# dgrzech/sobfu

Hardware: AMD Instinct MI355X
Metric: solver iterations/sec on 256^3 voxel grid (higher is better)
Workload: dtype f32

## Files before the change

### sobfu_amd/csrc/sobfu_launch.hpp

```cpp
#pragma once
#include <hip/hip_runtime.h>

#include <cstddef>
#include <cstdint>

namespace sobfu_hip {
struct LaunchBox {
    int x0, x1, y0, y1, z0, z1;
    bool direct;
};
struct TileLaunchBox {
    LaunchBox box;
    float* dst;
    int ox, oy, oz, px, py;
    int push_y0, push_y1, local_z0, local_z1;
};
int launch_pass_a_boxes(const float* pnp, const float* pg, const float* psi, float* nU, float w_reg, int X, int Y, int Z, const LaunchBox* boxes,
                        int n, const uint32_t* prev_slots, float max_update_norm, int zc, hipStream_t stream, bool compact);
constexpr int kMaxSync = 64;
struct TileSync {
    uint32_t ticket_push, reserved;
    uint64_t wait_ticks;
    uint32_t wait_count, pad0;
    uint32_t err;
    uint32_t n_sync;
    uint32_t my_rank, world;
    uint64_t timeout_ticks;
    uint32_t* my_flags;
    uint32_t* my_grows;
    int sync_rank[kMaxSync];
    uint32_t* peer_flags[kMaxSync];
    uint32_t* peer_grows[kMaxSync];
};
struct TilePassAPlan;
int tile_pass_a_plan_create(TilePassAPlan** out, const TileLaunchBox* boxes, int n, int X, int Y, int Z);
void tile_pass_a_plan_destroy(TilePassAPlan* p);
int launch_tile_pass_a_plan(const TilePassAPlan* p, const float* pnp, const float* pg, const float* psi, float* nU, float w_reg, TileSync* sync,
                            uint32_t seq, int wait, const uint32_t* row, uint32_t row_index, hipStream_t stream);
int launch_tile_flush(TileSync* sync, uint32_t seq, int wait, const uint32_t* row, uint32_t row_index, hipStream_t stream);
int launch_tile_pingpong(TileSync* sync, int q, int first, uint32_t seq0, int reps, hipStream_t stream);
int launch_pass_b_boxes(const float* nU, float* psi, const float* phi_n, float* pnp, float* updates, uint32_t* slots, const float taps[7],
                        float alpha, int X, int Y, int Z, int pX, int pY, int pZ, const int own[6], const LaunchBox* boxes, int n,
                        const uint32_t* prev_slots, float max_update_norm, int zc, hipStream_t stream, bool compact,
                        float* psi_out = nullptr , int prev_rows = 1,
                        bool sys_acquire = false );
int launch_pass_a(const float* pnp, const float* pg, const float* psi, float* nU, float w_reg, int X, int Y, int Z,
                  const uint32_t* prev_slots, float max_update_norm, int zc, hipStream_t stream, bool compact, int z_lo = 0, int z_hi = 0,
                  int z_lo2 = 0, int z_hi2 = 0);
int launch_pass_b(const float* nU, float* psi, const float* phi_n, float* pnp, float* updates, uint32_t* slots,
                  const float taps[7], float alpha, int X, int Y, int Z, const uint32_t* prev_slots,
                  float max_update_norm, int zc, hipStream_t stream, int phi_Z, int own_lo, int own_hi, bool compact, int z_lo = 0,
                  int z_hi = 0, int z_lo2 = 0, int z_hi2 = 0, float* psi_out = nullptr ,
                  int prev_rows = 1 );
int launch_pack_vec(const float* src4, float* dst3, size_t N, hipStream_t stream);
int launch_unpack_vec(const float* src3, float* dst4, size_t N, hipStream_t stream);
int launch_extract_tsdf(const float* src2, float* dst1, size_t N, hipStream_t stream);
int launch_apply_tsdf_only(const float* phi1, float* out1, const float* psi3, int X, int Y, int Z, hipStream_t stream, int phi_Z = 0, int phi_X = 0,
                           int phi_Y = 0);
int launch_msg_copy(bool pack, float* field3, float* buf, int Lx, int Ly, int Lz, const int* boxes, int n, hipStream_t stream);
int launch_msg_scatter_table(float* field3, const float* buf, const uint32_t* d_table, unsigned n_cells, hipStream_t stream);
int launch_compact_enter(const float* psi4, const float* pg2, const float* pn2, float* c_psi, float* c_g, float* c_n, float* c_f, int X, int Y,
                         int Z, hipStream_t stream);
int launch_compact_leave(const float* c_psi, const float* pn2, float* psi4, float* pnp2, int X, int Y, int Z, hipStream_t stream);
int data_energy_tsdf(const float* g1, const float* f1, int n, void* d_scratch, float* out, hipStream_t stream);
int reg_energy_from_psi3(const float* psi3, int X, int Y, int Z, void* d_scratch, float* out, hipStream_t stream);
}
```

### sobfu_amd/csrc/solver_capi.hip

```cpp
#include <algorithm>
#include <cmath>
#include <cstdio>
#include <cstdlib>
#include <cstring>
#include <string>
#include <vector>

#include "sobfu_device.hpp"
#include "sobfu_hip.h"
#include "sobfu_host.hpp"
#include "sobfu_launch.hpp"


namespace {

constexpr int kSlots      = 256;
constexpr int kCheckEvery = 32;
constexpr int kMaxRunAhead = 96;

float host_sqrt_rd(float s) {
    float r = std::sqrt(s);
    if (r > 0.f && (double) r * (double) r > (double) s) r = std::nextafterf(r, -INFINITY);
    return r;
}

float slots_to_norm(const uint32_t* s) {
    uint32_t m = 0;
    for (int i = 0; i < kSlots; ++i) m = s[i] > m ? s[i] : m;
    float f;
    std::memcpy(&f, &m, 4);
    return host_sqrt_rd(f);
}

}

struct sobfu_hip_solver {
    int X = 0, Y = 0, Z = 0;
    size_t N = 0;
    sobfu_hip_solver_params p{};
    float taps[7]{};
    float* nabla_U     = nullptr;
    float* updates     = nullptr;
    float* c_psi = nullptr;
    float* c_f   = nullptr;
    float* c_g   = nullptr;
    float* c_n   = nullptr;
    bool compact = true;
    uint32_t* slots    = nullptr;
    uint32_t* h_rows   = nullptr;
    int h_rows_iters   = 0;
    hipEvent_t ev_chk  = nullptr;
    void* red_scratch  = nullptr;
    int slots_iters    = 0;
    bool keep_updates  = false;
    sobfu_hip_log_fn log_fn = nullptr;
    void* log_user          = nullptr;
    bool log_set            = false;
    size_t bytes            = 0;
    int prof_stride = 0;
    std::vector<hipEvent_t> events;
    double ms_a = 0, ms_b = 0;
    int prof_launches = 0, prof_pending = 0;
    struct Session {
        bool active = false, compact = false;
        const float *pg = nullptr, *pn = nullptr;
        float *pnp = nullptr, *psi = nullptr;
        const float *it_pnp = nullptr, *it_pg = nullptr, *it_pn = nullptr;
        float *it_psi = nullptr, *it_out = nullptr, *upd = nullptr;
        int cap = 0;
        int launched = 0;
        int checked = 0, fl_to = 0;
        bool in_flight = false;
        int done = 0;
        bool converged = false;
        float last_norm = 0.f;
        bool inline_log = false;
    } q;

    void log(const std::string& line) const {
        if (log_set) {
            if (log_fn) log_fn(line.c_str(), log_user);
        } else {
            std::printf("%s\n", line.c_str());
        }
    }
};

namespace {

std::string fmt_g(float v) {
    char b[64];
    std::snprintf(b, sizeof b, "%g", (double) v);
    return b;
}

int ensure_slots(sobfu_hip_solver* s, int iters) {
    if (iters <= s->slots_iters) return 0;
    if (s->slots) {
        SOBFU_HIP_TRY(hipFree(s->slots));
        s->bytes -= (size_t) (s->slots_iters + 1) * kSlots * 4;
    }
    s->slots = nullptr;
    SOBFU_HIP_TRY(hipMalloc((void**) &s->slots, (size_t) (iters + 1) * kSlots * 4));
    s->slots_iters = iters;
    s->bytes += (size_t) (iters + 1) * kSlots * 4;
    return 0;
}

int ensure_poll(sobfu_hip_solver* s, int iters) {
    if (!s->ev_chk) SOBFU_HIP_TRY(hipEventCreateWithFlags(&s->ev_chk, hipEventDisableTiming));
    if (iters <= s->h_rows_iters) return 0;
    if (s->h_rows) SOBFU_HIP_TRY(hipHostFree(s->h_rows));
    s->h_rows = nullptr;
    SOBFU_HIP_TRY(hipHostMalloc((void**) &s->h_rows, (size_t) iters * kSlots * 4, hipHostMallocDefault));
    s->h_rows_iters = iters;
    return 0;
}

int ensure_compact(sobfu_hip_solver* s) {
    if (s->c_psi) return 0;
    SOBFU_HIP_TRY(hipMalloc((void**) &s->c_psi, s->N * 12));
    SOBFU_HIP_TRY(hipMalloc((void**) &s->c_f, s->N * 4));
    SOBFU_HIP_TRY(hipMalloc((void**) &s->c_g, s->N * 4));
    SOBFU_HIP_TRY(hipMalloc((void**) &s->c_n, s->N * 4));
    s->bytes += s->N * 24;
    return 0;
}

int ensure_updates(sobfu_hip_solver* s) {
    if (s->updates) return 0;
    SOBFU_HIP_TRY(hipMalloc((void**) &s->updates, s->N * 16));
    s->bytes += s->N * 16;
    return 0;
}

int set_params(sobfu_hip_solver* s, const sobfu_hip_solver_params* p) {
    SOBFU_CHECK_ARGS(p && p->max_iter >= 0);
    if (p->s < 7 || p->s > 16) return p->s < 7 ? SOBFU_E_UNSUPPORTED : SOBFU_E_FILTER;
    float h[16];
    SOBFU_TRY(sobfu_hip_sobolev_filter(p->s, p->lambda, h));
    for (int i = 0; i < 7; ++i) s->taps[i] = h[i];
    s->p = *p;
    return 0;
}

int ensure_events(sobfu_hip_solver* s, size_t n) {
    while (s->events.size() < n) {
        hipEvent_t e;
        SOBFU_HIP_TRY(hipEventCreate(&e));
        s->events.push_back(e);
    }
    return 0;
}

int session_begin_impl(sobfu_hip_solver* s, const float* pg, const float* pn, float* pnp, float* psi, int cap, hipStream_t st) {
    sobfu_hip_solver::Session& q = s->q;
    const int X = s->X, Y = s->Y, Z = s->Z;
    q = sobfu_hip_solver::Session{};
    q.pg = pg; q.pn = pn; q.pnp = pnp; q.psi = psi;
    q.cap = cap;
    q.compact = s->compact && cap > 0;
    q.last_norm = NAN;
    if (!q.compact) SOBFU_TRY(sobfu_hip_apply(pn, pnp, psi, X, Y, Z, st));
    if (cap <= 0) return 0;
    SOBFU_TRY(ensure_slots(s, cap));
    SOBFU_HIP_TRY(hipMemsetAsync(s->slots, 0, (size_t) (cap + 1) * kSlots * 4, st));
    if (s->keep_updates) {
        SOBFU_TRY(ensure_updates(s));
        q.upd = s->updates;
    }
    q.it_pnp = pnp; q.it_pg = pg; q.it_pn = pn; q.it_psi = psi; q.it_out = pnp;
    if (q.compact) {
        SOBFU_TRY(ensure_compact(s));
        SOBFU_TRY(sobfu_hip::launch_compact_enter(psi, pg, pn, s->c_psi, s->c_g, s->c_n, s->c_f, X, Y, Z, st));
        q.it_pnp = s->c_f; q.it_pg = s->c_g; q.it_pn = s->c_n; q.it_psi = s->c_psi; q.it_out = s->c_f;
    }
    if (s->p.max_update_norm >= 0.f) SOBFU_TRY(ensure_poll(s, cap));
    if (s->prof_stride > 0) SOBFU_TRY(ensure_events(s, (size_t) 3 * (cap / s->prof_stride + 1)));
    return 0;
}
int session_begin(sobfu_hip_solver* s, const float* pg, const float* pn, float* pnp, float* psi, int cap, hipStream_t st) {
    if (s->q.active) return SOBFU_E_BADARG;
    const int rc = session_begin_impl(s, pg, pn, pnp, psi, cap, st);
    s->q.active = rc == 0;
    return rc;
}

void session_examine(sobfu_hip_solver* s, int upto, float* per_iter) {
    sobfu_hip_solver::Session& q = s->q;
    for (int k = q.checked; k < upto && !q.converged; ++k) {
        const float v = slots_to_norm(s->h_rows + (size_t) k * kSlots);
        if (per_iter) per_iter[k] = v;
        q.last_norm = v;
        q.done = k + 1;
        if (v <= s->p.max_update_norm) q.converged = true;
    }
    q.checked = upto;
}

int session_enqueue(sobfu_hip_solver* s, int n, bool poll, float* per_iter, hipStream_t st) {
    sobfu_hip_solver::Session& q = s->q;
    if (!q.active || n < 0 || q.launched + n > q.cap) return SOBFU_E_BADARG;
    const int X = s->X, Y = s->Y, Z = s->Z;
    const sobfu_hip_solver_params& p = s->p;
    const bool can_converge = p.max_update_norm >= 0.f;
    const int last = q.launched + n;
    for (int it = q.launched + 1; it <= last && !q.converged; ++it) {
        const uint32_t* prev = (it > 1) ? s->slots + (size_t) (it - 1) * kSlots : nullptr;
        uint32_t* cur        = s->slots + (size_t) it * kSlots;
        const bool ev = s->prof_stride > 0 && (it % s->prof_stride == 0) && (size_t) 3 * (s->prof_pending + 1) <= s->events.size();
        const int e0  = 3 * s->prof_pending;
        if (ev) SOBFU_HIP_TRY(hipEventRecord(s->events[e0], st));
        SOBFU_TRY(sobfu_hip::launch_pass_a(q.it_pnp, q.it_pg, q.it_psi, s->nabla_U, p.w_reg, X, Y, Z, prev, p.max_update_norm, 0, st, q.compact));
        if (ev) SOBFU_HIP_TRY(hipEventRecord(s->events[e0 + 1], st));
        SOBFU_TRY(sobfu_hip::launch_pass_b(s->nabla_U, q.it_psi, q.it_pn, q.it_out, q.upd, cur, s->taps, p.alpha, X, Y, Z, prev,
                                           p.max_update_norm, 0, st, 0, 0, 0, q.compact));
        if (ev) {
            SOBFU_HIP_TRY(hipEventRecord(s->events[e0 + 2], st));
            s->prof_pending += 1;
        }
        q.launched = it;
        if (can_converge && poll) {
            if (!q.in_flight && (it % kCheckEvery == 0 || it == last)) {
                SOBFU_HIP_TRY(hipMemcpyAsync(s->h_rows + (size_t) q.checked * kSlots, s->slots + (size_t) (q.checked + 1) * kSlots,
                                             (size_t) (it - q.checked) * kSlots * 4, hipMemcpyDeviceToHost, st));
                SOBFU_HIP_TRY(hipEventRecord(s->ev_chk, st));
                q.in_flight = true;
                q.fl_to     = it;
            }
            if (q.in_flight) {
                const bool must_wait = it - q.checked >= kMaxRunAhead;
                hipError_t e = must_wait ? hipEventSynchronize(s->ev_chk) : hipEventQuery(s->ev_chk);
                if (e == hipSuccess) {
                    session_examine(s, q.fl_to, per_iter);
                    q.in_flight = false;
                } else if (e != hipErrorNotReady) {
                    return (int) e;
                }
            }
        }
    }
    return 0;
}

int session_drain(sobfu_hip_solver* s, float* per_iter, hipStream_t st) {
    sobfu_hip_solver::Session& q = s->q;
    if (q.launched == 0) return 0;
    if (s->p.max_update_norm >= 0.f) {
        if (q.in_flight) {
            SOBFU_HIP_TRY(hipEventSynchronize(s->ev_chk));
            session_examine(s, q.fl_to, per_iter);
            q.in_flight = false;
        }
        if (!q.converged && q.checked < q.launched) {
            SOBFU_HIP_TRY(hipMemcpyAsync(s->h_rows + (size_t) q.checked * kSlots, s->slots + (size_t) (q.checked + 1) * kSlots,
                                         (size_t) (q.launched - q.checked) * kSlots * 4, hipMemcpyDeviceToHost, st));
            SOBFU_HIP_TRY(hipStreamSynchronize(st));
            session_examine(s, q.launched, per_iter);
        }
    } else {
        std::vector<uint32_t> hs((size_t) q.launched * kSlots);
        SOBFU_HIP_TRY(hipMemcpyAsync(hs.data(), s->slots + kSlots, hs.size() * 4, hipMemcpyDeviceToHost, st));
        SOBFU_HIP_TRY(hipStreamSynchronize(st));
        for (int k = 0; k < q.launched; ++k) {
            const float v = slots_to_norm(hs.data() + (size_t) k * kSlots);
            if (per_iter) per_iter[k] = v;
            q.last_norm = v;
        }
        q.done = q.launched;
    }
    return 0;
}

int session_end(sobfu_hip_solver* s, sobfu_hip_solver_report* rep, float* per_iter, hipStream_t st) {
    sobfu_hip_solver::Session& q = s->q;
    if (!q.active) return SOBFU_E_BADARG;
    sobfu_hip_solver_report r{};
    r.last_max_update_norm = NAN;
    r.last_max_update_index = NAN;
    r.last_e_data = r.last_e_reg = NAN;
    SOBFU_TRY(session_drain(s, per_iter, st));
    if (q.compact) SOBFU_TRY(sobfu_hip::launch_compact_leave(s->c_psi, q.pn, q.psi, q.pnp, s->X, s->Y, s->Z, st));
    for (int it = 1; it <= q.done && !q.inline_log; ++it)
        if (it == 1 || it % 50 == 0) s->log("iter. no. " + std::to_string(it));
    if (q.converged) s->log("SOLVER CONVERGED AFTER " + std::to_string(q.done) + " ITERATIONS");
    else if (q.cap > 0 && q.done == q.cap) s->log("SOLVER REACHED MAX. NO. OF ITERATIONS WITHOUT CONVERGING");
    r.iterations = q.done;
    r.converged  = q.converged ? 1 : 0;
    r.last_max_update_norm = q.last_norm;
    q.active = false;
    SOBFU_HIP_TRY(hipStreamSynchronize(st));
    if (rep) *rep = r;
    return 0;
}

int run_verbose(sobfu_hip_solver* s, const float* pg, const float* pn, float* pnp, float* psi, int max_iter,
                sobfu_hip_solver_report* rep, float* per_iter, hipStream_t st) {
    const int X = s->X, Y = s->Y, Z = s->Z;
    const sobfu_hip_solver_params& p = s->p;
    auto reports = [&](int it) { return p.verbosity == 2 || (p.verbosity == 1 && (it == 1 || it % 50 == 0 || it == max_iter)); };
    SOBFU_TRY(ensure_updates(s));
    SOBFU_TRY(session_begin(s, pg, pn, pnp, psi, max_iter, st));
    sobfu_hip_solver::Session& q = s->q;
    q.upd = s->updates;
    q.inline_log = p.verbosity <= 2;
    float e_data = NAN, e_reg = NAN, arg = NAN;
    auto fail = [&](int rc) {
        q.active = false;
        return rc;
    };
#define SOBFU_VTRY(expr)                    \
    do {                                    \
        const int rc_ = (int) (expr);       \
        if (rc_ != 0) return fail(rc_);     \
    } while (0)
    for (int it = 1; it <= max_iter && !q.converged;) {
        if (!reports(it)) {
            int to = it;
            while (to + 1 <= max_iter && !reports(to + 1)) ++to;
            SOBFU_VTRY(session_enqueue(s, to - it + 1, true, per_iter, st));
            if (p.max_update_norm >= 0.f) SOBFU_VTRY(session_drain(s, per_iter, st));
            it = to + 1;
            continue;
        }
        if (it == 1 || it % 50 == 0) s->log("iter. no. " + std::to_string(it));
        if (q.compact) {
            SOBFU_VTRY(sobfu_hip::data_energy_tsdf(q.it_pg, q.it_pnp, (int) s->N, s->red_scratch, &e_data, st));
            SOBFU_VTRY(sobfu_hip::reg_energy_from_psi3(q.it_psi, X, Y, Z, s->red_scratch, &e_reg, st));
        } else {
            SOBFU_VTRY(sobfu_hip_data_energy(pg, pnp, (int) s->N, s->red_scratch, &e_data, st));
            SOBFU_VTRY(sobfu_hip_reg_energy_sobolev_from_psi(psi, X, Y, Z, s->red_scratch, &e_reg, st));
        }
        const float e = e_data + p.w_reg * e_reg;
        s->log("data energy + w_reg * reg energy = " + fmt_g(e_data) + " + " + fmt_g(p.w_reg) + " * " + fmt_g(e_reg) + " = " + fmt_g(e));
        uint32_t* cur = s->slots + (size_t) it * kSlots;
        SOBFU_VTRY(sobfu_hip::launch_pass_a(q.it_pnp, q.it_pg, q.it_psi, s->nabla_U, p.w_reg, X, Y, Z, nullptr, 0.f, 0, st, q.compact));
        SOBFU_VTRY(sobfu_hip::launch_pass_b(s->nabla_U, q.it_psi, q.it_pn, q.it_out, s->updates, cur, s->taps, p.alpha, X, Y, Z, nullptr, 0.f, 0, st, 0,
                                            0, 0, q.compact));
        float mx[2];
        SOBFU_VTRY(sobfu_hip_max_update_norm(s->updates, (int) s->N, s->red_scratch, mx, st));
        if (per_iter) per_iter[it - 1] = mx[0];
        arg = mx[1];
        q.launched = q.checked = q.done = it;
        q.last_norm = mx[0];
        {
            int ix = (int) (mx[1] / (float) (X * Y));
            int iy = (int) ((mx[1] - (float) (ix * X * Y)) / (float) X);
            int iz = (int) (mx[1] - (float) (X * (iy + Y * ix)));
            s->log("max. update norm " + fmt_g(mx[0]) + " at voxel (" + std::to_string(iz) + ", " + std::to_string(iy) + ", " + std::to_string(ix) + ")");
        }
        if (mx[0] <= p.max_update_norm) q.converged = true;
        ++it;
    }
#undef SOBFU_VTRY
    const bool last_reported = q.done > 0 && reports(q.done);
    sobfu_hip_solver_report r{};
    SOBFU_TRY(session_end(s, &r, per_iter, st));
    r.last_e_data = e_data;
    r.last_e_reg  = e_reg;
    r.last_max_update_index = last_reported ? arg : NAN;
    if (rep) *rep = r;
    return 0;
}

int run_loop(sobfu_hip_solver* s, const float* pg, const float* pn, float* pnp, float* psi, int max_iter,
             sobfu_hip_solver_report* rep, float* per_iter, hipStream_t st) {
    if (s->q.active) return SOBFU_E_BADARG;
    if (s->p.verbosity > 0 && max_iter > 0) return run_verbose(s, pg, pn, pnp, psi, max_iter, rep, per_iter, st);
    SOBFU_TRY(session_begin(s, pg, pn, pnp, psi, max_iter, st));
// ... 192 lines not shown
```

### sobfu_amd/csrc/solver_kernels.hip

```cpp
#include <algorithm>
#include <cstdlib>
#include <vector>

#include "sobfu_device.hpp"
#include "sobfu_hip.h"
#include "sobfu_host.hpp"
#include "sobfu_launch.hpp"

using namespace sobfu_hip;

#ifndef SOBFU_SWIZZLE_B
#define SOBFU_SWIZZLE_B true
#endif

namespace {

struct Taps {
    float s[7];
};
constexpr int kMaxMsgs = 18;

#include "solver_iter_common.inl"
#include "solver_pass_a.inl"
#include "solver_pass_b.inl"
#include "solver_aux_kernels.inl"

}

constexpr int kRPT = 1, kWY = 8;

namespace sobfu_hip {

static int env_zc(const char* env) {
    const char* e = getenv(env);
    const int v   = e ? atoi(e) : 0;
    return v > 0 ? v : 0;
}
int pick_zc(int X, int Y, int nz, int ty, int capacity, int refill, const char* env) {
    if (const int v = env_zc(env)) return v < nz ? v : nz;
    const long tiles = (long) ((X + TX - 1) / TX) * ((Y + ty - 1) / ty);
    int best_zc = nz;
    double best = 1e30;
    for (int c = 1; c <= nz; ++c) {
        const int zc = (nz + c - 1) / c;
        if (zc < 2 && nz >= 2) break;
        const long groups = tiles * ((nz + zc - 1) / zc);
        const long waves  = (groups + capacity - 1) / capacity;
        const double util = (double) groups / (double) (waves * capacity);
        const double cost = (1.0 + (double) refill / zc) / util;
        if (cost < best - 1e-9) { best = cost; best_zc = zc; }
    }
    return best_zc;
}

static bool cache_resident(int X, int Y, int Z) {
    const char* e = getenv("SOBFU_CACHE_CELLS");
    return (long) X * Y * Z <= (e ? atol(e) : 3300000L);
}

static int direct_wx(int ex) {
    int wx = 1;
    while (wx < ex && wx < 64) wx *= 2;
    return wx;
}
static int direct_wpg(int wx, bool spread) { return spread ? std::max(1, std::min(kWY, wx / 4)) : kWY; }
static int direct_groups(const LaunchBox& s, int wx, bool spread) {
    const int wyl = 64 / wx, wpg = direct_wpg(wx, spread);
    const long waves = (long) ((s.x1 - s.x0 + wx - 1) / wx) * ((s.y1 - s.y0 + wyl - 1) / wyl) * (s.z1 - s.z0);
    return (int) ((waves + wpg - 1) / wpg);
}
static double box_cells(const LaunchBox& s) {
    return (s.x1 > s.x0 && s.y1 > s.y0 && s.z1 > s.z0) ? (double) (s.x1 - s.x0) * (s.y1 - s.y0) * (s.z1 - s.z0) : 0.0;
}
static int finish_box(Box& b, const LaunchBox& s, int ty, int share, int refill, int zc_override, const char* env, bool spread, bool even = false) {
    b.x0 = s.x0; b.x1 = s.x1; b.y0 = s.y0; b.y1 = s.y1; b.z0 = s.z0; b.z1 = s.z1;
    b.kind = s.direct ? 1 : 0;
    b.wpg = kWY;
    b.rem = 0;
    b.pair = 0;
    if (s.direct) {
        b.zc  = direct_wx(s.x1 - s.x0);
        b.wpg = direct_wpg(b.zc, spread);
        return direct_groups(s, b.zc, spread);
    }
    const int eu = s.x1 - s.x0, ev = s.y1 - s.y0, nz = s.z1 - s.z0;
    const int tiles = ((eu + TX - 1) / TX) * ((ev + ty - 1) / ty);
    int nch = 0;
    if (zc_override <= 0 && env_zc(env) == 0 && even && tiles <= share) nch = std::max(share / tiles, 1);
    if (nch > 0 && zc_override <= 0) {
        nch   = std::min(nch, std::max(nz / 2, 1));
        b.zc  = nz / nch;
        b.rem = nz % nch;
        return tiles * nch;
    }
    b.zc = zc_override > 0 ? std::min(zc_override, nz) : pick_zc(eu, ev, nz, ty, share, refill, env);
    return tiles * ((nz + b.zc - 1) / b.zc);
}
static int finish_boxes(BoxList& L, const LaunchBox* boxes, int n, int ty, int capacity, int refill, int zc_override, const char* env,
                        bool even = false) {
    L.n = 0;
    int live = 0;
    bool thin = false;
    for (int i = 0; i < n; ++i) {
        live += (box_cells(boxes[i]) > 0 && !boxes[i].direct) ? 1 : 0;
        thin = thin || (box_cells(boxes[i]) > 0 && boxes[i].direct);
    }
    if (even && thin) capacity -= capacity / 16;
    int total = 0;
    L.m0 = L.m1 = 0;
    for (int pass = 0; pass < 2; ++pass) {
        const bool direct_pass = pass == 1;
        if (!direct_pass) L.m0 = total;
        for (int i = 0; i < n && L.n < kMaxBoxes; ++i) {
            if (box_cells(boxes[i]) == 0 || boxes[i].direct != direct_pass) continue;
            L.first[L.n] = total;
            total += finish_box(L.b[L.n], boxes[i], ty, std::max(capacity / std::max(live, 1), 1), refill, zc_override, env, true, even);
            ++L.n;
        }
        if (!direct_pass) L.m1 = total;
    }
    for (int k = L.n; k <= kMaxBoxes; ++k) L.first[k] = total;
    return total;
}

static int fill_tile_boxes(TileBoxList& L, const TileLaunchBox* boxes, int n, int X, int Y, int Z, int zc) {
    constexpr int TY = kRPT * kWY;
    L.n = 0;
    int live = 0, total = 0;
    for (int i = 0; i < n; ++i) live += (box_cells(boxes[i].box) > 0 && !boxes[i].box.direct && boxes[i].dst == nullptr) ? 1 : 0;
    for (int pass = 0; pass < 2; ++pass) {
        for (int i = 0; i < n; ++i) {
            const TileLaunchBox& s = boxes[i];
            if ((s.dst != nullptr) != (pass == 0) || box_cells(s.box) == 0) continue;
            if (L.n >= kMaxTileBoxes) return -1;
            TileBox& t = L.b[L.n];
            L.first[L.n] = total;
            const int zc_box = zc > 0 ? zc : ((s.dst != nullptr && !s.box.direct) ? std::min(8, s.box.z1 - s.box.z0) : 0);
            total += finish_box(t.b, s.box, TY, std::max(256 * (cache_resident(X, Y, Z) ? 2 : 4) * 8 / kWY / std::max(live, 1), 1), 2, zc_box,
                                "SOBFU_ZC_A", false);
            t.push.base = s.dst;
            t.push.ox = s.ox; t.push.oy = s.oy; t.push.oz = s.oz; t.push.px = s.px; t.push.py = s.py;
            t.push.y0 = s.push_y0; t.push.y1 = s.push_y1; t.push.lz0 = s.local_z0; t.push.lz1 = s.local_z1;
            ++L.n;
        }
        if (pass == 0) L.n_push_wgs = total;
    }
    for (int k = L.n; k <= kMaxTileBoxes; ++k) L.first[k] = total;
    return total;
}

static int launch_tile_boxes(const TileBoxList* d_boxes, int groups, const float* pnp, const float* pg, const float* psi, float* nU, float w_reg, int X,
                             int Y, int Z, TileSync* sync, uint32_t seq, int wait, const uint32_t* row, uint32_t row_index, hipStream_t stream,
                             bool compact) {
    if (groups == 0) return 0;
    TilePassAArgsP a{{pnp, pg, psi, nU, {X, Y, Z}, w_reg, nullptr, 0.f}, d_boxes, {sync, seq, wait, row, row_index}};
    const dim3 grid((unsigned) groups), block(TX, kWY);
    if (compact && cache_resident(X, Y, Z)) hipLaunchKernelGGL((tile_potential_gradient_kernel<kRPT, kWY, true, 0>), grid, block, 0, stream, a);
    else if (compact) hipLaunchKernelGGL((tile_potential_gradient_kernel<kRPT, kWY, true, kNT>), grid, block, 0, stream, a);
    else hipLaunchKernelGGL((tile_potential_gradient_kernel<kRPT, kWY, false, 0>), grid, block, 0, stream, a);
    return (int) hipGetLastError();
}

int launch_pass_a_boxes(const float* pnp, const float* pg, const float* psi, float* nU, float w_reg, int X, int Y, int Z, const LaunchBox* boxes,
                        int n, const uint32_t* prev_slots, float max_update_norm, int zc, hipStream_t stream, bool compact) {
    constexpr int TY = kRPT * kWY;
    bool direct = false;
    for (int i = 0; i < n; ++i) direct = direct || (boxes[i].direct && box_cells(boxes[i]) > 0);
    if (direct) {
        std::vector<TileLaunchBox> tb((size_t) n);
        for (int i = 0; i < n; ++i) tb[(size_t) i] = TileLaunchBox{boxes[i], nullptr, 0, 0, 0, 0, 0, 0, 0, 0, 0};
        TileBoxList L{};
        const int total = fill_tile_boxes(L, tb.data(), n, X, Y, Z, zc);
        if (total <= 0) return total < 0 ? SOBFU_E_BADARG : 0;
        TileBoxList* d = nullptr;
        SOBFU_HIP_TRY(hipMallocAsync((void**) &d, sizeof L, stream));
        const hipError_t e = hipMemcpyAsync(d, &L, sizeof L, hipMemcpyHostToDevice, stream);
        const int rc = e != hipSuccess ? (int) e : launch_tile_boxes(d, total, pnp, pg, psi, nU, w_reg, X, Y, Z, nullptr, 0, 0, nullptr, 0, stream, compact);
        const hipError_t f = hipFreeAsync(d, stream);
        return rc != 0 ? rc : (int) f;
    }
    PassAArgs a{{pnp, pg, psi, nU, {X, Y, Z}, w_reg, prev_slots, max_update_norm}, {}};
    const int groups = finish_boxes(a.boxes, boxes, n, TY, 256 * 4 * 8 / kWY, 2, zc, "SOBFU_ZC_A");
    if (groups == 0) return 0;
    const dim3 grid((unsigned) groups), block(TX, kWY);
    if (compact && cache_resident(X, Y, Z)) hipLaunchKernelGGL((fused_potential_gradient_kernel<kRPT, kWY, true, 0>), grid, block, 0, stream, a);
    else if (compact) hipLaunchKernelGGL((fused_potential_gradient_kernel<kRPT, kWY, true, kNT>), grid, block, 0, stream, a);
    else hipLaunchKernelGGL((fused_potential_gradient_kernel<kRPT, kWY, false, 0>), grid, block, 0, stream, a);
    return (int) hipGetLastError();
}

struct TilePassAPlan {
    TileBoxList* d_boxes = nullptr;
    int groups = 0, X = 0, Y = 0, Z = 0;
};
int tile_pass_a_plan_create(TilePassAPlan** out, const TileLaunchBox* boxes, int n, int X, int Y, int Z) {
    TileBoxList L{};
    const int total = fill_tile_boxes(L, boxes, n, X, Y, Z, 0);
    if (total < 0) return SOBFU_E_BADARG;
    auto* p = new TilePassAPlan();
    p->groups = total; p->X = X; p->Y = Y; p->Z = Z;
    hipError_t e = hipSuccess;
    if (total > 0) {
        e = hipMalloc((void**) &p->d_boxes, sizeof L);
        if (e == hipSuccess) e = hipMemcpy(p->d_boxes, &L, sizeof L, hipMemcpyHostToDevice);
    }
    if (e != hipSuccess) {
        if (p->d_boxes) (void) hipFree(p->d_boxes);
        delete p;
        return (int) e;
    }
    *out = p;
    return 0;
}
void tile_pass_a_plan_destroy(TilePassAPlan* p) {
    if (p == nullptr) return;
    if (p->d_boxes) (void) hipFree(p->d_boxes);
    delete p;
}
int launch_tile_pass_a_plan(const TilePassAPlan* p, const float* pnp, const float* pg, const float* psi, float* nU, float w_reg, TileSync* sync,
                            uint32_t seq, int wait, const uint32_t* row, uint32_t row_index, hipStream_t stream) {
    return launch_tile_boxes(p->d_boxes, p->groups, pnp, pg, psi, nU, w_reg, p->X, p->Y, p->Z, sync, seq, wait, row, row_index, stream, true);
}

int launch_tile_pingpong(TileSync* sync, int q, int first, uint32_t seq0, int reps, hipStream_t stream) {
    hipLaunchKernelGGL(tile_pingpong_kernel, dim3(1), dim3(64), 0, stream, sync, q, first, seq0, reps);
    return (int) hipGetLastError();
}

int launch_tile_flush(TileSync* sync, uint32_t seq, int wait, const uint32_t* row, uint32_t row_index, hipStream_t stream) {
    hipLaunchKernelGGL(tile_flush_kernel, dim3(1), dim3(64), 0, stream, sync, seq, wait, row, row_index);
    return (int) hipGetLastError();
}

int launch_pass_b_boxes(const float* nU, float* psi, const float* phi_n, float* pnp, float* updates, uint32_t* slots, const float taps[7],
                        float alpha, int X, int Y, int Z, int pX, int pY, int pZ, const int own[6], const LaunchBox* boxes, int n,
                        const uint32_t* prev_slots, float max_update_norm, int zc, hipStream_t stream, bool compact, float* psi_out, int prev_rows,
                        bool sys_acquire) {
    constexpr int TY = kRPT * kWY;
    PassBArgs a{nU, psi, phi_n, pnp, (float4*) updates, slots, {X, Y, Z}, {}, alpha, {}, prev_slots, max_update_norm, {pX, pY, pZ},
                {own[0], own[1], own[2], own[3], own[4], own[5]}, prev_rows, psi_out ? psi_out : psi, sys_acquire ? 1 : 0};
    for (int i = 0; i < 7; ++i) a.S.s[i] = taps[i];
    if ((size_t) X * Y * 16 >= ((size_t) 1 << 32)) return SOBFU_E_UNSUPPORTED;
    if (sys_acquire && (size_t) X * Y * Z * 12 >= ((size_t) 1 << 32)) return SOBFU_E_UNSUPPORTED;
    const bool idx32 = (size_t) pX * pY * pZ < ((size_t) 1 << 30);
    const bool resident = cache_resident(X, Y, Z);
    const char* pipe_e = getenv("SOBFU_PIPE_B");
    const bool pipe = compact && idx32 && !updates && (size_t) X * Y * Z * 12 < ((size_t) 1 << 32) && (sys_acquire || (pipe_e ? atoi(pipe_e) != 0 : resident));
    if (sys_acquire && !pipe) return SOBFU_E_UNSUPPORTED;
    const int groups = finish_boxes(a.boxes, boxes, n, TY, 256 * (pipe ? 2 : 3) * 8 / kWY, 6, zc, "SOBFU_ZC_B", resident && pipe);
    if (groups == 0) return 0;
    bool direct = false;
    int zc_max = 0;
    for (int i = 0; i < a.boxes.n; ++i) {
        direct = direct || a.boxes.b[i].kind != 0;
        if (a.boxes.b[i].kind == 0) zc_max = std::max(zc_max, a.boxes.b[i].zc + (a.boxes.b[i].rem > 0 ? 1 : 0));
        if (a.boxes.b[i].kind == 0 && pipe && resident && SOBFU_PAIR_B) a.boxes.b[i].pair = 1;
    }
    const dim3 grid((unsigned) groups), block(TX, kWY);
#define SOBFU_LAUNCH_B(UPD, CMP, DIR) \
    hipLaunchKernelGGL((fused_smooth_update_apply_kernel<kRPT, kWY, UPD, CMP, DIR>), grid, block, 0, stream, a)
#define SOBFU_LAUNCH_BX(DIR, HLV, NTV, PIP) \
    hipLaunchKernelGGL((fused_smooth_update_apply_kernel<kRPT, kWY, false, true, DIR, true, HLV, NTV, PIP>), grid, block, 0, stream, a)
    const bool ntbuf = (size_t) X * Y * Z * 12 < ((size_t) 1 << 32);
    if (direct) {
        if (updates && compact) SOBFU_LAUNCH_B(true, true, true);
        else if (updates) SOBFU_LAUNCH_B(true, false, true);
        else if (compact && idx32) {
            if (resident && pipe) SOBFU_LAUNCH_BX(true, 0, 0, true);
            else if (resident) SOBFU_LAUNCH_BX(true, 0, 0, false);
            else if (pipe) SOBFU_LAUNCH_BX(true, 0, kNT, true);
            else if (ntbuf) hipLaunchKernelGGL((fused_smooth_update_apply_kernel<kRPT, kWY, false, true, true, true, 0, kNT, false, true>), grid, block, 0, stream, a);
            else SOBFU_LAUNCH_BX(true, 0, kNT, false);
        }
        else if (compact) SOBFU_LAUNCH_B(false, true, true);
        else SOBFU_LAUNCH_B(false, false, true);
    } else {
        if (updates && compact) SOBFU_LAUNCH_B(true, true, false);
        else if (updates) SOBFU_LAUNCH_B(true, false, false);
        else if (compact && idx32) {
            const bool lead = SOBFU_HLEAD > 0 && zc_max >= SOBFU_HLEAD_MIN_ZC && !resident && !pipe;
            if (lead && ntbuf) hipLaunchKernelGGL((fused_smooth_update_apply_kernel<kRPT, kWY, false, true, false, true, SOBFU_HLEAD, kNT, false, true>), grid, block, 0, stream, a);
            else if (lead) SOBFU_LAUNCH_BX(false, SOBFU_HLEAD, kNT, false);
            else if (resident && pipe) SOBFU_LAUNCH_BX(false, 0, 0, true);
            else if (resident) SOBFU_LAUNCH_BX(false, 0, 0, false);
            else if (pipe) SOBFU_LAUNCH_BX(false, 0, kNT, true);
            else if (ntbuf) hipLaunchKernelGGL((fused_smooth_update_apply_kernel<kRPT, kWY, false, true, false, true, 0, kNT, false, true>), grid, block, 0, stream, a);
            else SOBFU_LAUNCH_BX(false, 0, kNT, false);
        }
        else if (compact) SOBFU_LAUNCH_B(false, true, false);
        else SOBFU_LAUNCH_B(false, false, false);
    }
#undef SOBFU_LAUNCH_BX
#undef SOBFU_LAUNCH_B
    return (int) hipGetLastError();
}

int launch_pass_a(const float* pnp, const float* pg, const float* psi, float* nU, float w_reg, int X, int Y, int Z,
                  const uint32_t* prev_slots, float max_update_norm, int zc, hipStream_t stream, bool compact, int z_lo, int z_hi,
                  int z_lo2, int z_hi2) {
    if (z_hi <= 0 && z_hi2 <= z_lo2) { z_lo = 0; z_hi = Z; }
    const LaunchBox b[2] = {{0, X, 0, Y, z_lo, z_hi, false}, {0, X, 0, Y, z_lo2, z_hi2, false}};
    return launch_pass_a_boxes(pnp, pg, psi, nU, w_reg, X, Y, Z, b, 2, prev_slots, max_update_norm, zc, stream, compact);
}

int launch_pass_b(const float* nU, float* psi, const float* phi_n, float* pnp, float* updates, uint32_t* slots,
                  const float taps[7], float alpha, int X, int Y, int Z, const uint32_t* prev_slots,
                  float max_update_norm, int zc, hipStream_t stream, int phi_Z, int own_lo, int own_hi, bool compact, int z_lo,
                  int z_hi, int z_lo2, int z_hi2, float* psi_out, int prev_rows) {
    if (phi_Z <= 0) { phi_Z = Z; own_lo = 0; own_hi = Z; }
    if (z_hi <= 0 && z_hi2 <= z_lo2) { z_lo = 0; z_hi = Z; }
    const LaunchBox b[2] = {{0, X, 0, Y, z_lo, z_hi, false}, {0, X, 0, Y, z_lo2, z_hi2, false}};
    const int own[6] = {0, X, 0, Y, own_lo, own_hi};
    return launch_pass_b_boxes(nU, psi, phi_n, pnp, updates, slots, taps, alpha, X, Y, Z, X, Y, phi_Z, own, b, 2, prev_slots, max_update_norm, zc,
                               stream, compact, psi_out, prev_rows);
}

#define SOBFU_LIN(N) dim3((unsigned) (((N) + 255) / 256)), dim3(256), 0, stream
int launch_pack_vec(const float* src4, float* dst3, size_t N, hipStream_t stream) {
    hipLaunchKernelGGL(pack_vec_kernel, SOBFU_LIN(N), (const float4*) src4, (P3*) dst3, N);
    return (int) hipGetLastError();
}
int launch_unpack_vec(const float* src3, float* dst4, size_t N, hipStream_t stream) {
    hipLaunchKernelGGL(unpack_vec_kernel, SOBFU_LIN(N), (const P3*) src3, (float4*) dst4, N);
    return (int) hipGetLastError();
}
int launch_extract_tsdf(const float* src2, float* dst1, size_t N, hipStream_t stream) {
    hipLaunchKernelGGL(extract_tsdf_kernel, SOBFU_LIN(N), (const float2*) src2, dst1, N);
    return (int) hipGetLastError();
}
int launch_apply_tsdf_only(const float* phi1, float* out1, const float* psi3, int X, int Y, int Z, hipStream_t stream, int phi_Z, int phi_X,
                           int phi_Y) {
    hipLaunchKernelGGL(apply_tsdf_only_kernel, voxel_grid(X, Y, Z), voxel_block(), 0, stream, phi1, out1, (const P3*) psi3, Dims{X, Y, Z},
                       Dims{phi_X > 0 ? phi_X : X, phi_Y > 0 ? phi_Y : Y, phi_Z > 0 ? phi_Z : Z});
    return (int) hipGetLastError();
}
int launch_msg_copy(bool pack, float* field3, float* buf, int Lx, int Ly, int Lz, const int* boxes, int n, hipStream_t stream) {
    if (n <= 0) return 0;
    if (n > kMaxMsgs) return SOBFU_E_BADARG;
    MsgBoxes m{};
    m.n = n;
    unsigned total = 0;
    for (int i = 0; i < n; ++i) {
        const int* b = boxes + 6 * i;
        if (!(b[0] >= 0 && b[1] > b[0] && b[1] <= Lx && b[2] >= 0 && b[3] > b[2] && b[3] <= Ly && b[4] >= 0 && b[5] > b[4] && b[5] <= Lz)) return SOBFU_E_BADARG;
        m.x0[i] = b[0]; m.y0[i] = b[2]; m.z0[i] = b[4];
        m.nx[i] = b[1] - b[0]; m.ny[i] = b[3] - b[2];
        m.first[i] = total;
        total += (unsigned) (b[1] - b[0]) * (unsigned) (b[3] - b[2]) * (unsigned) (b[5] - b[4]);
    }
    for (int k = n; k <= kMaxMsgs; ++k) m.first[k] = total;
    const dim3 grid((total + 255u) / 256u), block(256);
    if (pack) hipLaunchKernelGGL(msg_copy_kernel<true>, grid, block, 0, stream, field3, buf, Dims{Lx, Ly, Lz}, m);
    else hipLaunchKernelGGL(msg_copy_kernel<false>, grid, block, 0, stream, field3, buf, Dims{Lx, Ly, Lz}, m);
    return (int) hipGetLastError();
}
int launch_msg_scatter_table(float* field3, const float* buf, const uint32_t* d_table, unsigned n_cells, hipStream_t stream) {
    if (n_cells == 0) return 0;
    hipLaunchKernelGGL(msg_scatter_table_kernel, dim3((n_cells + 255u) / 256u), dim3(256), 0, stream, field3, buf, d_table, n_cells);
    return (int) hipGetLastError();
}
#undef SOBFU_LIN
int launch_compact_enter(const float* psi4, const float* pg2, const float* pn2, float* c_psi, float* c_g, float* c_n, float* c_f, int X, int Y,
                         int Z, hipStream_t stream) {
    hipLaunchKernelGGL(compact_enter_kernel, voxel_grid(X, Y, Z), voxel_block(), 0, stream, (const float4*) psi4, (const float2*) pg2,
                       (const float2*) pn2, (P3*) c_psi, c_g, c_n, c_f, Dims{X, Y, Z});
    return (int) hipGetLastError();
}
int launch_compact_leave(const float* c_psi, const float* pn2, float* psi4, float* pnp2, int X, int Y, int Z, hipStream_t stream) {
    hipLaunchKernelGGL(compact_leave_kernel, voxel_grid(X, Y, Z), voxel_block(), 0, stream, (const P3*) c_psi, (const float2*) pn2,
                       (float4*) psi4, (float2*) pnp2, Dims{X, Y, Z});
    return (int) hipGetLastError();
}

}

extern "C" {

int sobfu_hip_fused_potential_gradient(const float* d_phi_n_psi, const float* d_phi_global, const float* d_psi,
                                       float* d_nabla_U, float w_reg, int X, int Y, int Z, void* stream) {
    SOBFU_CHECK_ARGS(d_phi_n_psi && d_phi_global && d_psi && d_nabla_U && X > 1 && Y > 1 && Z > 1);
    if ((size_t) X * Y * Z > (size_t) 0x7fffffff) return SOBFU_E_UNSUPPORTED;
    return sobfu_hip::launch_pass_a(d_phi_n_psi, d_phi_global, d_psi, d_nabla_U, w_reg, X, Y, Z, nullptr, 0.f, 0, (hipStream_t) stream, false, 0, 0);
}

int sobfu_hip_fused_smooth_update_apply(const float* d_nabla_U, float* d_psi, const float* d_phi_n, float* d_phi_n_psi,
                                        float* d_updates, uint32_t* d_max_sq_slots, const float taps[7], float alpha,
                                        int X, int Y, int Z, void* stream) {
    SOBFU_CHECK_ARGS(d_nabla_U && d_psi && d_phi_n && d_phi_n_psi && d_max_sq_slots && taps && X > 0 && Y > 0 && Z > 0);
    if ((size_t) X * Y * Z > (size_t) 0x7fffffff) return SOBFU_E_UNSUPPORTED;
    return sobfu_hip::launch_pass_b(d_nabla_U, d_psi, d_phi_n, d_phi_n_psi, d_updates, d_max_sq_slots, taps, alpha, X, Y, Z,
                                    nullptr, 0.f, 0, (hipStream_t) stream, 0, 0, 0, false, 0, 0);
}

int sobfu_hip_pack_vec3(const float* d_src4, float* d_dst3, size_t n, void* stream) {
    SOBFU_CHECK_ARGS(d_src4 && d_dst3 && n > 0);
    return sobfu_hip::launch_pack_vec(d_src4, d_dst3, n, (hipStream_t) stream);
}
int sobfu_hip_unpack_vec3(const float* d_src3, float* d_dst4, size_t n, void* stream) {
    SOBFU_CHECK_ARGS(d_src3 && d_dst4 && n > 0);
    return sobfu_hip::launch_unpack_vec(d_src3, d_dst4, n, (hipStream_t) stream);
}
int sobfu_hip_extract_tsdf(const float* d_src2, float* d_dst1, size_t n, void* stream) {
    SOBFU_CHECK_ARGS(d_src2 && d_dst1 && n > 0);
    return sobfu_hip::launch_extract_tsdf(d_src2, d_dst1, n, (hipStream_t) stream);
}
static bool box_ok(const int b[6], int Lx, int Ly, int Lz) {
    return b[0] >= 0 && b[0] <= b[1] && b[1] <= Lx && b[2] >= 0 && b[2] <= b[3] && b[3] <= Ly && b[4] >= 0 && b[4] <= b[5] && b[5] <= Lz;
}

int sobfu_hip_tile3_potential_gradient(const float* d_phi_n_psi, const float* d_phi_global, const float* d_psi, float* d_nabla_U, float w_reg,
                                       int Lx, int Ly, int Lz, const int box[6], int thin, const uint32_t* d_prev_slots,
                                       float max_update_norm, int compact, void* stream) {
    SOBFU_CHECK_ARGS(d_phi_n_psi && d_phi_global && d_psi && d_nabla_U && Lx > 1 && Ly > 1 && Lz > 1 && box && box_ok(box, Lx, Ly, Lz));
    if ((size_t) Lx * Ly * Lz > (size_t) 0x7fffffff) return SOBFU_E_UNSUPPORTED;
    const sobfu_hip::LaunchBox b{box[0], box[1], box[2], box[3], box[4], box[5], thin != 0};
    return sobfu_hip::launch_pass_a_boxes(d_phi_n_psi, d_phi_global, d_psi, d_nabla_U, w_reg, Lx, Ly, Lz, &b, 1, d_prev_slots, max_update_norm, 0,
                                          (hipStream_t) stream, compact != 0);
}

int sobfu_hip_tile3_smooth_update_apply(const float* d_nabla_U, float* d_psi, const float* d_phi_n, float* d_phi_n_psi, float* d_updates,
                                        uint32_t* d_max_sq_slots, const float taps[7], float alpha, int Lx, int Ly, int Lz, int Xg, int Yg,
                                        int Zg, const int own[6], const int box[6], int thin, const uint32_t* d_prev_slots,
                                        float max_update_norm, int compact, void* stream) {
    SOBFU_CHECK_ARGS(d_nabla_U && d_psi && d_phi_n && d_phi_n_psi && d_max_sq_slots && taps && Lx > 0 && Ly > 0 && Lz > 0 && Xg > 0 && Yg > 0 &&
                     Zg > 0 && own && box && box_ok(own, Lx, Ly, Lz) && box_ok(box, Lx, Ly, Lz));
    if ((size_t) Lx * Ly * Lz > (size_t) 0x7fffffff || (size_t) Xg * Yg * Zg > (size_t) 0x7fffffff) return SOBFU_E_UNSUPPORTED;
    const sobfu_hip::LaunchBox b{box[0], box[1], box[2], box[3], box[4], box[5], thin != 0};
    return sobfu_hip::launch_pass_b_boxes(d_nabla_U, d_psi, d_phi_n, d_phi_n_psi, d_updates, d_max_sq_slots, taps, alpha, Lx, Ly, Lz, Xg, Yg, Zg,
                                          own, &b, 1, d_prev_slots, max_update_norm, 0, (hipStream_t) stream, compact != 0);
}

int sobfu_hip_tile3_apply_tsdf_only(const float* d_phi1, int Xg, int Yg, int Zg, float* d_out1, const float* d_psi3, int Lx, int Ly, int Lz,
                                    void* stream) {
    SOBFU_CHECK_ARGS(d_phi1 && d_out1 && d_psi3 && Lx > 0 && Ly > 0 && Lz > 0 && Xg > 0 && Yg > 0 && Zg > 0);
    return sobfu_hip::launch_apply_tsdf_only(d_phi1, d_out1, d_psi3, Lx, Ly, Lz, (hipStream_t) stream, Zg, Xg, Yg);
}

int sobfu_hip_tile3_pack(const float* d_field3, int Lx, int Ly, int Lz, float* d_buf, const int* boxes, int n_boxes, void* stream) {
    SOBFU_CHECK_ARGS(d_field3 && d_buf && boxes && n_boxes >= 0 && Lx > 0 && Ly > 0 && Lz > 0);
    return sobfu_hip::launch_msg_copy(true, const_cast<float*>(d_field3), d_buf, Lx, Ly, Lz, boxes, n_boxes, (hipStream_t) stream);
}

int sobfu_hip_tile3_unpack(float* d_field3, int Lx, int Ly, int Lz, const float* d_buf, const int* boxes, int n_boxes, void* stream) {
    SOBFU_CHECK_ARGS(d_field3 && d_buf && boxes && n_boxes >= 0 && Lx > 0 && Ly > 0 && Lz > 0);
    return sobfu_hip::launch_msg_copy(false, d_field3, const_cast<float*>(d_buf), Lx, Ly, Lz, boxes, n_boxes, (hipStream_t) stream);
}

}
```

Baseline: 4055.

## Move warp/apply step from pass B into pass A in compact loop

```diff
diff --git a/sobfu_amd/csrc/sobfu_launch.hpp b/sobfu_amd/csrc/sobfu_launch.hpp
--- a/sobfu_amd/csrc/sobfu_launch.hpp
+++ b/sobfu_amd/csrc/sobfu_launch.hpp
@@ -16,7 +16,8 @@
     int push_y0, push_y1, local_z0, local_z1;
 };
 int launch_pass_a_boxes(const float* pnp, const float* pg, const float* psi, float* nU, float w_reg, int X, int Y, int Z, const LaunchBox* boxes,
-                        int n, const uint32_t* prev_slots, float max_update_norm, int zc, hipStream_t stream, bool compact);
+                        int n, const uint32_t* prev_slots, float max_update_norm, int zc, hipStream_t stream, bool compact,
+                        bool warp = false );
 constexpr int kMaxSync = 64;
 struct TileSync {
     uint32_t ticket_push, reserved;
@@ -43,15 +44,17 @@
                         float alpha, int X, int Y, int Z, int pX, int pY, int pZ, const int own[6], const LaunchBox* boxes, int n,
                         const uint32_t* prev_slots, float max_update_norm, int zc, hipStream_t stream, bool compact,
                         float* psi_out = nullptr , int prev_rows = 1,
-                        bool sys_acquire = false );
+                        bool sys_acquire = false ,
+                        bool apply = true );
 int launch_pass_a(const float* pnp, const float* pg, const float* psi, float* nU, float w_reg, int X, int Y, int Z,
                   const uint32_t* prev_slots, float max_update_norm, int zc, hipStream_t stream, bool compact, int z_lo = 0, int z_hi = 0,
-                  int z_lo2 = 0, int z_hi2 = 0);
+                  int z_lo2 = 0, int z_hi2 = 0, bool warp = false);
 int launch_pass_b(const float* nU, float* psi, const float* phi_n, float* pnp, float* updates, uint32_t* slots,
                   const float taps[7], float alpha, int X, int Y, int Z, const uint32_t* prev_slots,
                   float max_update_norm, int zc, hipStream_t stream, int phi_Z, int own_lo, int own_hi, bool compact, int z_lo = 0,
                   int z_hi = 0, int z_lo2 = 0, int z_hi2 = 0, float* psi_out = nullptr ,
-                  int prev_rows = 1 );
+                  int prev_rows = 1 , bool apply = true);
+bool loop_warps_in_pass_a(int X, int Y, int Z);
 int launch_pack_vec(const float* src4, float* dst3, size_t N, hipStream_t stream);
 int launch_unpack_vec(const float* src3, float* dst4, size_t N, hipStream_t stream);
 int launch_extract_tsdf(const float* src2, float* dst1, size_t N, hipStream_t stream);
diff --git a/sobfu_amd/csrc/solver_capi.hip b/sobfu_amd/csrc/solver_capi.hip
--- a/sobfu_amd/csrc/solver_capi.hip
+++ b/sobfu_amd/csrc/solver_capi.hip
@@ -75,6 +75,7 @@
         bool converged = false;
         float last_norm = 0.f;
         bool inline_log = false;
+        bool warp = false;
     } q;
 
     void log(const std::string& line) const {
@@ -174,6 +175,7 @@
         SOBFU_TRY(ensure_compact(s));
         SOBFU_TRY(sobfu_hip::launch_compact_enter(psi, pg, pn, s->c_psi, s->c_g, s->c_n, s->c_f, X, Y, Z, st));
         q.it_pnp = s->c_f; q.it_pg = s->c_g; q.it_pn = s->c_n; q.it_psi = s->c_psi; q.it_out = s->c_f;
+        q.warp = s->p.verbosity == 0 && !q.upd && sobfu_hip::loop_warps_in_pass_a(X, Y, Z);
     }
     if (s->p.max_update_norm >= 0.f) SOBFU_TRY(ensure_poll(s, cap));
     if (s->prof_stride > 0) SOBFU_TRY(ensure_events(s, (size_t) 3 * (cap / s->prof_stride + 1)));
@@ -211,10 +213,11 @@
         const bool ev = s->prof_stride > 0 && (it % s->prof_stride == 0) && (size_t) 3 * (s->prof_pending + 1) <= s->events.size();
         const int e0  = 3 * s->prof_pending;
         if (ev) SOBFU_HIP_TRY(hipEventRecord(s->events[e0], st));
-        SOBFU_TRY(sobfu_hip::launch_pass_a(q.it_pnp, q.it_pg, q.it_psi, s->nabla_U, p.w_reg, X, Y, Z, prev, p.max_update_norm, 0, st, q.compact));
+        SOBFU_TRY(sobfu_hip::launch_pass_a(q.warp ? q.it_pn : q.it_pnp, q.it_pg, q.it_psi, s->nabla_U, p.w_reg, X, Y, Z, prev, p.max_update_norm, 0,
+                                           st, q.compact, 0, 0, 0, 0, q.warp));
         if (ev) SOBFU_HIP_TRY(hipEventRecord(s->events[e0 + 1], st));
         SOBFU_TRY(sobfu_hip::launch_pass_b(s->nabla_U, q.it_psi, q.it_pn, q.it_out, q.upd, cur, s->taps, p.alpha, X, Y, Z, prev,
-                                           p.max_update_norm, 0, st, 0, 0, 0, q.compact));
+                                           p.max_update_norm, 0, st, 0, 0, 0, q.compact, 0, 0, 0, 0, nullptr, 1, !q.warp));
         if (ev) {
             SOBFU_HIP_TRY(hipEventRecord(s->events[e0 + 2], st));
             s->prof_pending += 1;
diff --git a/sobfu_amd/csrc/solver_kernels.hip b/sobfu_amd/csrc/solver_kernels.hip
--- a/sobfu_amd/csrc/solver_kernels.hip
+++ b/sobfu_amd/csrc/solver_kernels.hip
@@ -161,11 +161,20 @@
     return (int) hipGetLastError();
 }
 
+bool loop_warps_in_pass_a(int X, int Y, int Z) {
+    const char* e = getenv("SOBFU_WARP_A");
+    if (e && atoi(e) == 0) return false;
+    const char* pipe_e = getenv("SOBFU_PIPE_B");
+    const size_t n = (size_t) X * Y * Z;
+    return !cache_resident(X, Y, Z) && !(pipe_e && atoi(pipe_e) != 0) && n * 12 < ((size_t) 1 << 32) && (size_t) X * Y * 16 < ((size_t) 1 << 32);
+}
+
 int launch_pass_a_boxes(const float* pnp, const float* pg, const float* psi, float* nU, float w_reg, int X, int Y, int Z, const LaunchBox* boxes,
-                        int n, const uint32_t* prev_slots, float max_update_norm, int zc, hipStream_t stream, bool compact) {
+                        int n, const uint32_t* prev_slots, float max_update_norm, int zc, hipStream_t stream, bool compact, bool warp) {
     constexpr int TY = kRPT * kWY;
     bool direct = false;
     for (int i = 0; i < n; ++i) direct = direct || (boxes[i].direct && box_cells(boxes[i]) > 0);
+    if (warp && (direct || !compact || cache_resident(X, Y, Z) || (size_t) X * Y * Z * 4 >= ((size_t) 1 << 32))) return SOBFU_E_UNSUPPORTED;
     if (direct) {
         std::vector<TileLaunchBox> tb((size_t) n);
         for (int i = 0; i < n; ++i) tb[(size_t) i] = TileLaunchBox{boxes[i], nullptr, 0, 0, 0, 0, 0, 0, 0, 0, 0};
@@ -183,7 +192,8 @@
     const int groups = finish_boxes(a.boxes, boxes, n, TY, 256 * 4 * 8 / kWY, 2, zc, "SOBFU_ZC_A");
     if (groups == 0) return 0;
     const dim3 grid((unsigned) groups), block(TX, kWY);
-    if (compact && cache_resident(X, Y, Z)) hipLaunchKernelGGL((fused_potential_gradient_kernel<kRPT, kWY, true, 0>), grid, block, 0, stream, a);
+    if (warp) hipLaunchKernelGGL((fused_potential_gradient_kernel<kRPT, kWY, true, kNT, true>), grid, block, 0, stream, a);
+    else if (compact && cache_resident(X, Y, Z)) hipLaunchKernelGGL((fused_potential_gradient_kernel<kRPT, kWY, true, 0>), grid, block, 0, stream, a);
     else if (compact) hipLaunchKernelGGL((fused_potential_gradient_kernel<kRPT, kWY, true, kNT>), grid, block, 0, stream, a);
     else hipLaunchKernelGGL((fused_potential_gradient_kernel<kRPT, kWY, false, 0>), grid, block, 0, stream, a);
     return (int) hipGetLastError();
@@ -235,7 +245,7 @@
 int launch_pass_b_boxes(const float* nU, float* psi, const float* phi_n, float* pnp, float* updates, uint32_t* slots, const float taps[7],
                         float alpha, int X, int Y, int Z, int pX, int pY, int pZ, const int own[6], const LaunchBox* boxes, int n,
                         const uint32_t* prev_slots, float max_update_norm, int zc, hipStream_t stream, bool compact, float* psi_out, int prev_rows,
-                        bool sys_acquire) {
+                        bool sys_acquire, bool apply) {
     constexpr int TY = kRPT * kWY;
     PassBArgs a{nU, psi, phi_n, pnp, (float4*) updates, slots, {X, Y, Z}, {}, alpha, {}, prev_slots, max_update_norm, {pX, pY, pZ},
                 {own[0], own[1], own[2], own[3], own[4], own[5]}, prev_rows, psi_out ? psi_out : psi, sys_acquire ? 1 : 0};
@@ -256,12 +266,13 @@
         if (a.boxes.b[i].kind == 0) zc_max = std::max(zc_max, a.boxes.b[i].zc + (a.boxes.b[i].rem > 0 ? 1 : 0));
         if (a.boxes.b[i].kind == 0 && pipe && resident && SOBFU_PAIR_B) a.boxes.b[i].pair = 1;
     }
+    const bool ntbuf = (size_t) X * Y * Z * 12 < ((size_t) 1 << 32);
+    if (!apply && (direct || !compact || !idx32 || updates || resident || pipe || !ntbuf || sys_acquire)) return SOBFU_E_UNSUPPORTED;
     const dim3 grid((unsigned) groups), block(TX, kWY);
 #define SOBFU_LAUNCH_B(UPD, CMP, DIR) \
     hipLaunchKernelGGL((fused_smooth_update_apply_kernel<kRPT, kWY, UPD, CMP, DIR>), grid, block, 0, stream, a)
 #define SOBFU_LAUNCH_BX(DIR, HLV, NTV, PIP) \
     hipLaunchKernelGGL((fused_smooth_update_apply_kernel<kRPT, kWY, false, true, DIR, true, HLV, NTV, PIP>), grid, block, 0, stream, a)
-    const bool ntbuf = (size_t) X * Y * Z * 12 < ((size_t) 1 << 32);
     if (direct) {
         if (updates && compact) SOBFU_LAUNCH_B(true, true, true);
         else if (updates) SOBFU_LAUNCH_B(true, false, true);
@@ -279,7 +290,9 @@
         else if (updates) SOBFU_LAUNCH_B(true, false, false);
         else if (compact && idx32) {
             const bool lead = SOBFU_HLEAD > 0 && zc_max >= SOBFU_HLEAD_MIN_ZC && !resident && !pipe;
-            if (lead && ntbuf) hipLaunchKernelGGL((fused_smooth_update_apply_kernel<kRPT, kWY, false, true, false, true, SOBFU_HLEAD, kNT, false, true>), grid, block, 0, stream, a);
+            if (!apply && lead) hipLaunchKernelGGL((fused_smooth_update_apply_kernel<kRPT, kWY, false, true, false, true, SOBFU_HLEAD, kNT, false, true, false>), grid, block, 0, stream, a);
+            else if (!apply) hipLaunchKernelGGL((fused_smooth_update_apply_kernel<kRPT, kWY, false, true, false, true, 0, kNT, false, true, false>), grid, block, 0, stream, a);
+            else if (lead && ntbuf) hipLaunchKernelGGL((fused_smooth_update_apply_kernel<kRPT, kWY, false, true, false, true, SOBFU_HLEAD, kNT, false, true>), grid, block, 0, stream, a);
             else if (lead) SOBFU_LAUNCH_BX(false, SOBFU_HLEAD, kNT, false);
             else if (resident && pipe) SOBFU_LAUNCH_BX(false, 0, 0, true);
             else if (resident) SOBFU_LAUNCH_BX(false, 0, 0, false);
@@ -297,22 +310,22 @@
 
 int launch_pass_a(const float* pnp, const float* pg, const float* psi, float* nU, float w_reg, int X, int Y, int Z,
                   const uint32_t* prev_slots, float max_update_norm, int zc, hipStream_t stream, bool compact, int z_lo, int z_hi,
-                  int z_lo2, int z_hi2) {
+                  int z_lo2, int z_hi2, bool warp) {
     if (z_hi <= 0 && z_hi2 <= z_lo2) { z_lo = 0; z_hi = Z; }
     const LaunchBox b[2] = {{0, X, 0, Y, z_lo, z_hi, false}, {0, X, 0, Y, z_lo2, z_hi2, false}};
-    return launch_pass_a_boxes(pnp, pg, psi, nU, w_reg, X, Y, Z, b, 2, prev_slots, max_update_norm, zc, stream, compact);
+    return launch_pass_a_boxes(pnp, pg, psi, nU, w_reg, X, Y, Z, b, 2, prev_slots, max_update_norm, zc, stream, compact, warp);
 }
 
 int launch_pass_b(const float* nU, float* psi, const float* phi_n, float* pnp, float* updates, uint32_t* slots,
                   const float taps[7], float alpha, int X, int Y, int Z, const uint32_t* prev_slots,
                   float max_update_norm, int zc, hipStream_t stream, int phi_Z, int own_lo, int own_hi, bool compact, int z_lo,
-                  int z_hi, int z_lo2, int z_hi2, float* psi_out, int prev_rows) {
+                  int z_hi, int z_lo2, int z_hi2, float* psi_out, int prev_rows, bool apply) {
     if (phi_Z <= 0) { phi_Z = Z; own_lo = 0; own_hi = Z; }
     if (z_hi <= 0 && z_hi2 <= z_lo2) { z_lo = 0; z_hi = Z; }
     const LaunchBox b[2] = {{0, X, 0, Y, z_lo, z_hi, false}, {0, X, 0, Y, z_lo2, z_hi2, false}};
     const int own[6] = {0, X, 0, Y, own_lo, own_hi};
     return launch_pass_b_boxes(nU, psi, phi_n, pnp, updates, slots, taps, alpha, X, Y, Z, X, Y, phi_Z, own, b, 2, prev_slots, max_update_norm, zc,
-                               stream, compact, psi_out, prev_rows);
+                               stream, compact, psi_out, prev_rows, false, apply);
 }
 
 #define SOBFU_LIN(N) dim3((unsigned) (((N) + 255) / 256)), dim3(256), 0, stream
```

New measurement: 4332, median of 6. +6.8%, better.
